# johnmartinsson/differentiable-mel-spectrogram

Hardware: AMD Instinct MI355X
Metric: spectrogram frames/sec (fwd+bwd) (higher is better)
Workload: dtype f32

## Files before the change

differentiable-mel-spectrogram_amd/csrc/dmel_api.cpp:

```cpp
#include "../../include/dmel.h"
#include "dmel_kernels.h"

#include <algorithm>
#include <cmath>
#include <cstdio>
#include <cstdlib>
#include <cstring>
#include <functional>
#include <initializer_list>
#include <map>
#include <mutex>
#include <string>
#include <unordered_set>
#include <vector>

namespace {

thread_local std::string g_err;

dmel_status fail(dmel_status st, const std::string& msg)
{
    g_err = msg;
    return st;
}
// ... 494 lines not shown
                    const bool fin = pc.idx == 0;
                    for (int j = 0; j < 4; ++j) {
                        const int m = 4 * pc.quad + j;
                        lanes[(size_t)ph * 64 + 4 * b + j] = make_int2(8 * k0, (fin && m < M) ? m : -1);
                        merge[(size_t)ph * 64 + 4 * b + j] = (4 * p1 + j) | ((4 * p2 + j) << 8) | (f1 << 16) | (f2 << 17);
                        if (m >= M) continue;
                        for (int st = 0; st < 4 * n4; ++st) {
                            const int f = k0 + st;
                            const float v = (f < tb.F && f >= pc.lo && f < pc.lo + pc.w) ? fb[(size_t)f * M + m] : 0.f;
                            float4& e = b4[base + (size_t)(st / 4) * 64 + 4 * b + j];
                            (st % 4 == 0 ? e.x : st % 4 == 1 ? e.y : st % 4 == 2 ? e.z : e.w) = v;
                        }
                    }
                }
                tb.wl_mg[ph] = mg;
                tb.wl_total4 += n4;
            }
            DMEL_HIP(hipMalloc(&tb.wl_lane, lanes.size() * sizeof(int2)));
            DMEL_HIP(hipMemcpy(tb.wl_lane, lanes.data(), lanes.size() * sizeof(int2), hipMemcpyHostToDevice));
            DMEL_HIP(hipMalloc(&tb.wl_merge, merge.size() * sizeof(int)));
            DMEL_HIP(hipMemcpy(tb.wl_merge, merge.data(), merge.size() * sizeof(int), hipMemcpyHostToDevice));
            DMEL_HIP(hipMalloc(&tb.wl_b4, std::max<size_t>(b4.size(), 64) * sizeof(float4)));
            if (!b4.empty()) DMEL_HIP(hipMemcpy(tb.wl_b4, b4.data(), b4.size() * sizeof(float4), hipMemcpyHostToDevice));
        }
        {
            const int nbpre = dmel::forward_nbpre(N);
            std::vector<float> pre((size_t)waves * 2 * nbpre * 64, 0.f);
            for (int w = 0; w < waves; ++w)
                for (int loc = 0; loc < 2; ++loc) {
                    const int4 tr = ranges[(size_t)w * 2 + loc];
                    const int n = std::min(tr.y, nbpre);
                    tb.pre_groups[w * 2 + loc] = (n + 3) / 4;
                    if (n > 0)
                        std::copy(bfr.begin() + tr.z, bfr.begin() + tr.z + (size_t)n * 64, pre.begin() + ((size_t)(w * 2 + loc) * nbpre) * 64);
                }
            DMEL_HIP(hipMalloc(&tb.ent_pre, pre.size() * sizeof(float)));
            DMEL_HIP(hipMemcpy(tb.ent_pre, pre.data(), pre.size() * sizeof(float), hipMemcpyHostToDevice));
        }
        const size_t nb = std::max<size_t>(bfr.size(), 64);
        DMEL_HIP(hipMalloc(&tb.ent_b, nb * sizeof(float)));
        if (!bfr.empty())
            DMEL_HIP(hipMemcpy(tb.ent_b, bfr.data(), bfr.size() * sizeof(float), hipMemcpyHostToDevice));
        DMEL_HIP(hipMalloc(&tb.tile_ranges, ranges.size() * sizeof(int4)));
        DMEL_HIP(hipMemcpy(tb.tile_ranges, ranges.data(), ranges.size() * sizeof(int4), hipMemcpyHostToDevice));
    }
    auto ins = pl->tables.emplace(N, tb);
    guard.keep = true;
    *out = &ins.first->second;
    return DMEL_OK;
}

constexpr size_t kScratchPartials = 64, kScratchCounter = 64 + 8192, kScratchWin = 8320;
constexpr size_t kScratchPsum = kScratchWin + (size_t)dmel::kMaxNfft * 8;
static_assert(kScratchCounter - kScratchPartials == 1024 * sizeof(double) && dmel::kDotMaxBlocks * sizeof(double) == 4096 &&
              (dmel::kDotMaxBlocks / dmel::kDotGroup) * 64 <= 4096, "scratch layout the ticket tree relies on");

struct Scratch {
    unsigned* handled = nullptr; double* partials = nullptr; unsigned* counter = nullptr; float2* win = nullptr; float* psum = nullptr;
};

size_t scratch_bytes(const dmel_plan* pl, int batch)
{
    const size_t ps = ((size_t)std::max(batch, 1) * pl->nchunks * sizeof(float) + 255) / 256 * 256;
    return kScratchPsum + ps;
}

size_t scratch_bytes_multi(const dmel_plan* pl, int batch, int channels)
{
    return scratch_bytes(pl, batch) + (size_t)(channels - 1) * dmel::kMaxNfft * 8;
}

Scratch carve(void* base, int channels = 1)
{
    unsigned char* b = static_cast<unsigned char*>(base);
    Scratch sc;
    sc.handled = reinterpret_cast<unsigned*>(b);
    sc.partials = reinterpret_cast<double*>(b + kScratchPartials);
    sc.counter = reinterpret_cast<unsigned*>(b + kScratchCounter);
    sc.win = reinterpret_cast<float2*>(b + kScratchWin);
    sc.psum = reinterpret_cast<float*>(b + kScratchPsum + (size_t)(channels - 1) * dmel::kMaxNfft * 8);
    return sc;
}

bool is_capturing(hipStream_t s)
{
    hipStreamCaptureStatus st = hipStreamCaptureStatusNone;
    if (hipStreamIsCapturing(s, &st) != hipSuccess) { (void)hipGetLastError(); return false; }
    return st != hipStreamCaptureStatusNone;
}

dmel_status order_after_last_stream(dmel_plan* pl, hipStream_t s)
{
    if (pl->last_stream_valid && pl->last_stream != s && !is_capturing(s)) {
        if (hipEventRecord(pl->xev, pl->last_stream) == hipSuccess) DMEL_HIP(hipStreamWaitEvent(s, pl->xev, 0));
        else { (void)hipGetLastError(); DMEL_HIP(hipDeviceSynchronize()); }
    }
    pl->last_stream = s;
    pl->last_stream_valid = true;
    return DMEL_OK;
}

dmel_status ensure_own_scratch(dmel_plan* pl, int batch, hipStream_t s, Scratch* sc)
{
    if (!pl->own_scratch || batch > pl->own_scratch_clips) {
        if (is_capturing(s)) return fail(DMEL_ERR_INVALID_ARGUMENT, "plan scratch must grow but the stream is capturing: run one call eagerly first or pass scratch");
        if (pl->own_scratch) { DMEL_HIP(hipDeviceSynchronize()); (void)hipFree(pl->own_scratch); pl->own_scratch = nullptr; pl->own_scratch_clips = 0; }
        const int clips = std::max(batch, pl->cfg.max_batch);
// ... 2018 lines not shown
```

differentiable-mel-spectrogram_amd/csrc/dmel_aux.hip:

```cpp
#include <algorithm>
#include <cstdlib>
#include "dmel_kernels.h"
#include "dmel_ldsfft.h"

namespace dmel {

template <int CTRL> __device__ __forceinline__ double dpp_f64(double v)
{
    const long long b = __builtin_bit_cast(long long, v);
    const int lo = __builtin_amdgcn_mov_dpp((int)b, CTRL, 0xF, 0xF, true);
    const int hi = __builtin_amdgcn_mov_dpp((int)(b >> 32), CTRL, 0xF, 0xF, true);
    return __builtin_bit_cast(double, ((long long)hi << 32) | (unsigned)lo);
}
#ifndef DMEL_DOT_THREADS
#define DMEL_DOT_THREADS 256
#endif
constexpr int kDotThreads = DMEL_DOT_THREADS;
__device__ __forceinline__ double block_sum(double v, double* red4)
{
    v += dpp_f64<0xB1>(v);
    v += dpp_f64<0x4E>(v);
    v += dpp_f64<0x141>(v);
    v += dpp_f64<0x140>(v);
    const int tid = threadIdx.x;
    if ((tid & 15) == 0) red4[tid >> 4] = v;
    __syncthreads();
    double s = 0.0;
    for (int q = 0; q < kDotThreads / 16; ++q) s += red4[q];
    return s;
}

struct AdamConsts { float step, step_size, bc2_sqrt, omb1, omb2, b2, wd, eps; int maximize; };
__device__ __forceinline__ AdamConsts adam_consts(const AdamParams& p, float old_step)
{
    AdamConsts c;
    c.step = old_step + 1.0f;
    const float bc1 = (float)(1.0 - pow(p.beta1, (double)c.step)), bc2 = (float)(1.0 - pow(p.beta2, (double)c.step));
    c.step_size = (float)(p.lr / (double)bc1); c.bc2_sqrt = sqrtf(bc2);
    c.omb1 = (float)(1.0 - p.beta1); c.omb2 = (float)(1.0 - p.beta2); c.b2 = (float)p.beta2; c.wd = (float)p.weight_decay; c.eps = (float)p.eps;
    c.maximize = p.maximize;
    return c;
}
__device__ __forceinline__ void adam_update(const AdamParams& p, const AdamConsts& c, long long i, float g)
{
    const float w = p.param[i];
    if (c.maximize) g = -g;
    if (c.wd != 0.f) g = fmaf(w, c.wd, g);
    float m = p.exp_avg[i], v = p.exp_avg_sq[i];
    m = fmaf(c.omb1, g - m, m);
    v = fmaf(c.b2, v, c.omb2 * g * g);
    const float denom = sqrtf(v) / c.bc2_sqrt + c.eps;
    p.param[i] = w - c.step_size * m / denom;
    p.exp_avg[i] = m; p.exp_avg_sq[i] = v;
}

template <bool GBF16> __device__ __forceinline__ float4 load_g4(const void* g, long long i)
{
    if constexpr (!GBF16) return reinterpret_cast<const float4*>(g)[i];
    else {
        const uint2 v = reinterpret_cast<const uint2*>(g)[i];
        return make_float4(__uint_as_float(v.x << 16), __uint_as_float(v.x & 0xffff0000u),
                           __uint_as_float(v.y << 16), __uint_as_float(v.y & 0xffff0000u));
    }
}
template <bool GBF16> __device__ __forceinline__ float load_g1(const void* g, long long k)
{
    if constexpr (!GBF16) return reinterpret_cast<const float*>(g)[k];
    else return __uint_as_float((unsigned)reinterpret_cast<const unsigned short*>(g)[k] << 16);
}

__device__ __forceinline__ float mailbox_exchange(const MailboxArgs& mb, float local)
{
    const unsigned step = *mb.step + 1u;
    *mb.step = step;
    const unsigned long long mine = ((unsigned long long)step << 32) | __builtin_bit_cast(unsigned, local);
    const int par = (int)(step & 1u) * mb.world;
    for (int r = 0; r < mb.world; ++r)
        __hip_atomic_store(mb.peer_inbox[r] + par + mb.rank, mine, __ATOMIC_RELAXED, __HIP_MEMORY_SCOPE_SYSTEM);
    float sum = 0.f;
    bool ok = true;
    const unsigned long long t_start = __builtin_amdgcn_s_memrealtime();
    for (int r = 0; r < mb.world; ++r) {
        unsigned long long w = 0;
        unsigned spins = 0;
        for (;;) {
            w = __hip_atomic_load(mb.my_inbox + par + r, __ATOMIC_RELAXED, __HIP_MEMORY_SCOPE_SYSTEM);
            if ((unsigned)(w >> 32) == step) break;
            ++spins;
            if (mb.spin_limit && spins >= mb.spin_limit) { ok = false; break; }
            if (mb.timeout_ticks && (spins & 63u) == 0u && __builtin_amdgcn_s_memrealtime() - t_start >= mb.timeout_ticks) { ok = false; break; }
            if (spins < 4096u) __builtin_amdgcn_s_sleep(2); else __builtin_amdgcn_s_sleep(32);
        }
        if (!ok) {
            if (mb.host_error)
                __hip_atomic_store(mb.host_error, ((unsigned long long)step << 32) | (unsigned)r, __ATOMIC_RELAXED, __HIP_MEMORY_SCOPE_SYSTEM);
            return __builtin_nanf("");
        }
        sum += __builtin_bit_cast(float, (unsigned)w);
    }
    return sum;
}

__global__ void __launch_bounds__(64) dmel_mailbox_kernel(float* buf, MailboxArgs mb)
{
    if (threadIdx.x == 0) buf[0] = mailbox_exchange(mb, buf[0]);
}

hipError_t launch_mailbox_allreduce(float* buf, const MailboxArgs& mb, hipStream_t s)
{
    hipLaunchKernelGGL(dmel_mailbox_kernel, dim3(1), dim3(64), 0, s, buf, mb);
    return hipGetLastError();
}

template <bool GBF16, bool MBOX>
__global__ void __launch_bounds__(kDotThreads) dmel_dot_kernel(const void* __restrict__ g, const float* __restrict__ t,
                                                            long long count, double* partials, unsigned* counter,
                                                            int accumulate, float* result, MailboxArgs mb, AdamParams adam)
{
    __shared__ double red4[kDotThreads / 16], red4b[kDotThreads / 16];
    __shared__ int is_last;
    const int tid = threadIdx.x;
    const long long stride = (long long)gridDim.x * kDotThreads;
    double acc = 0.0;
    const uintptr_t galign = GBF16 ? 7 : 15;
    const long long n4 = ((reinterpret_cast<uintptr_t>(g) & galign) | (reinterpret_cast<uintptr_t>(t) & 15)) == 0 ? count / 4 : 0;
    const float4* t4 = reinterpret_cast<const float4*>(t);
    long long i = (long long)blockIdx.x * kDotThreads + tid;
    for (; i + 3 * stride < n4; i += 4 * stride) {
        const float4 a0 = load_g4<GBF16>(g, i), a1 = load_g4<GBF16>(g, i + stride), a2 = load_g4<GBF16>(g, i + 2 * stride), a3 = load_g4<GBF16>(g, i + 3 * stride);
        const float4 b0 = t4[i], b1 = t4[i + stride], b2 = t4[i + 2 * stride], b3 = t4[i + 3 * stride];
        acc += ((double)a0.x * (double)b0.x + (double)a0.y * (double)b0.y) + ((double)a0.z * (double)b0.z + (double)a0.w * (double)b0.w);
        acc += ((double)a1.x * (double)b1.x + (double)a1.y * (double)b1.y) + ((double)a1.z * (double)b1.z + (double)a1.w * (double)b1.w);
        acc += ((double)a2.x * (double)b2.x + (double)a2.y * (double)b2.y) + ((double)a2.z * (double)b2.z + (double)a2.w * (double)b2.w);
        acc += ((double)a3.x * (double)b3.x + (double)a3.y * (double)b3.y) + ((double)a3.z * (double)b3.z + (double)a3.w * (double)b3.w);
    }
    for (; i < n4; i += stride) {
        const float4 a = load_g4<GBF16>(g, i), b = t4[i];
        acc += ((double)a.x * (double)b.x + (double)a.y * (double)b.y) + ((double)a.z * (double)b.z + (double)a.w * (double)b.w);
    }
    for (long long k = n4 * 4 + (long long)blockIdx.x * kDotThreads + tid; k < count; k += stride)
        acc += (double)load_g1<GBF16>(g, k) * (double)t[k];
    const double bsum = block_sum(acc, red4);
    if (tid == 0) {
        __hip_atomic_store(&partials[blockIdx.x], bsum, __ATOMIC_RELAXED, __HIP_MEMORY_SCOPE_AGENT);
        asm volatile("s_waitcnt vmcnt(0)" ::: "memory");
        const unsigned grp = blockIdx.x / kDotGroup, ngroups = (gridDim.x + kDotGroup - 1) / kDotGroup;
        const unsigned gsize = grp + 1 < ngroups ? (unsigned)kDotGroup : gridDim.x - grp * kDotGroup;
        unsigned* gc = dot_group_counters(counter) + 16 * grp;
        bool last = false;
        if (__hip_atomic_fetch_add(gc, 1u, __ATOMIC_RELAXED, __HIP_MEMORY_SCOPE_AGENT) == gsize - 1u) {
            __hip_atomic_store(gc, 0u, __ATOMIC_RELAXED, __HIP_MEMORY_SCOPE_AGENT);
            last = __hip_atomic_fetch_add(counter, 1u, __ATOMIC_RELAXED, __HIP_MEMORY_SCOPE_AGENT) == ngroups - 1u;
        }
        is_last = last;
    }
    __syncthreads();
    if (!is_last) return;
    double sum = 0.0;
    for (int q = tid; q < (int)gridDim.x; q += kDotThreads)
        sum += __hip_atomic_load(&partials[q], __ATOMIC_RELAXED, __HIP_MEMORY_SCOPE_AGENT);
    const double total = block_sum(sum, red4b);
    if (tid == 0) {
        __hip_atomic_store(counter, 0u, __ATOMIC_RELAXED, __HIP_MEMORY_SCOPE_AGENT);
        if constexpr (MBOX) {
            const float all = mailbox_exchange(mb, (float)total);
            result[0] = accumulate ? result[0] + all : all;
        } else {
            result[0] = accumulate ? (float)((double)result[0] + total) : (float)total;
        }
        if (adam.param) {
            const AdamConsts c = adam_consts(adam, *adam.step);
            adam_update(adam, c, 0, result[0]);
            *adam.step = c.step;
        }
    }
}

int dot_blocks_for(long long count, int max_partials)
{
    static const long long per_wg = [] { const char* e = std::getenv("DMEL_DOT_PER_WG"); const long long v = e ? std::atoll(e) : 0; return v >= 1024 ? v : 4096LL; }();
    const long long want = (count + per_wg - 1) / per_wg;
    const long long cap = max_partials < kDotMaxBlocks ? max_partials : kDotMaxBlocks;
    return (int)(want < 1 ? 1 : (want > cap ? cap : want));
}

hipError_t launch_dot(const void* g, int g_bf16, const float* t, long long count, int accumulate, double* partials,
                      unsigned* counter, int max_partials, float* result, hipStream_t s, const MailboxArgs* mb, const AdamParams* fused)
{
    const int blocks = dot_blocks_for(count, max_partials);
    const MailboxArgs none{};
    AdamParams adam{};
    if (fused) adam = *fused;
    const dim3 gr(blocks), bl(kDotThreads);
    if (mb) {
        if (g_bf16) hipLaunchKernelGGL((dmel_dot_kernel<true, true>), gr, bl, 0, s, g, t, count, partials, counter, accumulate, result, *mb, adam);
        else hipLaunchKernelGGL((dmel_dot_kernel<false, true>), gr, bl, 0, s, g, t, count, partials, counter, accumulate, result, *mb, adam);
    } else {
        if (g_bf16) hipLaunchKernelGGL((dmel_dot_kernel<true, false>), gr, bl, 0, s, g, t, count, partials, counter, accumulate, result, none, adam);
        else hipLaunchKernelGGL((dmel_dot_kernel<false, false>), gr, bl, 0, s, g, t, count, partials, counter, accumulate, result, none, adam);
    }
    return hipGetLastError();
}

static_assert(kDotMaxBlocks * sizeof(double) == 4096 && kMaxChannels <= kDotMaxBlocks,
              "the multi dot writes at most kDotMaxBlocks partials: the ticket tree's group counters live in the upper half of the 1024");
template <bool GBF16>
__global__ void __launch_bounds__(kDotThreads) dmel_dot_multi_kernel(const void* __restrict__ g, const float* __restrict__ t, int K,
                                                                  unsigned rows_b, unsigned per_row, int bpc, double* partials,
                                                                  unsigned* counter, int accumulate, float* result)
{
    __shared__ double red4[kDotThreads / 16];
    __shared__ int is_last;
    const int tid = threadIdx.x;
    const int c = blockIdx.x / bpc, j = blockIdx.x - c * bpc;
    const unsigned stride = (unsigned)bpc * kDotThreads;
    double acc = 0.0;
// ... 203 lines not shown
#pragma unroll
            for (int u = 0; u < 4; ++u) {
                const long long i = ((long long)blk * 4 + u) * 256 + tid;
                if (i < n) {
                    p.fb_dense[i] = v[u];
                    if (p.fbT) { const int f = (int)(i / p.M), m = (int)(i % p.M); p.fbT[(size_t)m * p.F + f] = v[u]; }
                }
            }
            return;
        }
        blk -= p.blocks_c;
        const long long f = (long long)blk * 256 + tid;
        if (p.rowpk && f < p.F)
            p.rowpk[f] = make_float4(p.fb[f * p.M], p.M > 1 ? p.fb[f * p.M + 1] : 0.f, __builtin_bit_cast(float, 0), __builtin_bit_cast(float, p.M));
        if (p.ent_h && f < p.M) p.fb_nyq[f] = p.fb[(size_t)(p.F - 1) * p.M + f];
        return;
    }
    const int run = blockIdx.x / kRepackRunSplit, part = blockIdx.x % kRepackRunSplit;
    const int4 tr = p.tile_ranges[run];
    if (tr.y <= 0 || tr.w < 0) return;
    for (int i = part * 256 + tid; i < tr.y * 64; i += 256 * kRepackRunSplit) {
        const int ks = tr.x + i / 64, l = i % 64;
        const int f = 4 * ks + (l >> 4), m = 16 * (tr.w & 0xffff) + (l & 15);
        const float v = (f < p.F && m < p.M) ? p.fb[(size_t)f * p.M + m] : 0.f;
        p.ent_b[tr.z + i] = v;
        if (run < p.runs_group0 && i / 64 < p.nbpre) p.ent_pre[((size_t)run * p.nbpre + i / 64) * 64 + l] = v;
    }
}

hipError_t launch_repack(const RepackParams& p0, hipStream_t s)
{
    RepackParams p = p0;
    const long long n = (long long)p.F * p.M;
    const int NT = (p.M + 15) / 16;
    p.blocks_h = p.ent_h ? (int)(((long long)NT * p.ks32 * 64 + 255) / 256) : 0;
    p.blocks_w = p.wl_b4 ? (int)(((long long)p.wl_total4 * 64 + 255) / 256) : 0;
    p.blocks_c = (int)((n + 1023) / 1024);
    const int blocks_r = (std::max(p.F, p.M) + 255) / 256;
    hipLaunchKernelGGL(dmel_repack_kernel, dim3((unsigned)(p.runs * kRepackRunSplit + p.blocks_h + p.blocks_w + p.blocks_c + blocks_r)), dim3(256), 0, s, p);
    return hipGetLastError();
}

__global__ void __launch_bounds__(128) dmel_naive_kernel(NaiveParams p)
{
    extern __shared__ __attribute__((aligned(16))) unsigned char smem_raw[];
    float* fa = reinterpret_cast<float*>(smem_raw);
    float* fb_ = fa + p.N;
    float* P = fb_ + p.N;
    float* D = P + p.F;
    const int tid = threadIdx.x;
    const int b = blockIdx.x / p.T, t = blockIdx.x % p.T;
    const float* xb = resolve_x(p.x, p.x_ind) + (size_t)b * p.L;
    const bool spec_mode = (p.mode == kSpec || p.mode == kSpecTrain);
    const LamState ls = lam_prologue(p.lam, p.N, blockIdx.x == 0 && tid == 0);
    if (ls.action != kLamRun) {
        if (ls.action == kLamPoison) {
            const int rows = spec_mode ? p.F : p.M;
            for (int rr = tid; rr < rows; rr += blockDim.x) {
                const size_t o = ((size_t)b * rows + rr) * p.T + t;
                if (p.flags & 4u) reinterpret_cast<unsigned short*>(p.out)[o] = 0x7fc0u; else p.out[o] = __builtin_nanf("");
                if (p.tangent) p.tangent[o] = __builtin_nanf("");
            }
        }
        return;
    }
    const float ctan = lam_tangent_scale(ls);
    float mean = 0.f;
    if (p.remove_dc) {
        mean = clip_mean_psum(p.psum, p.nchunks, b, p.L);
    }
    for (int n = tid; n < p.N; n += blockDim.x) {
        const long long i = (long long)t * p.hop - p.N / 2 + n;
        const float v = (i >= 0 && i < p.L) ? (xb[i] - mean) : 0.f;
        const float2 wd = p.win2[n];
        fa[n] = v * wd.x;
        fb_[n] = v * wd.y;
    }
    __syncthreads();
    for (int f = tid; f < p.F; f += blockDim.x) {
        float xr = 0.f, xi = 0.f, yr = 0.f, yi = 0.f;
        for (int n = 0; n < p.N; ++n) {
            const int kn = (int)(((long long)f * n) % p.N);
            float sn, cs;
            sincospif(2.0f * (float)kn / (float)p.N, &sn, &cs);
            xr = fmaf(fa[n], cs, xr); xi = fmaf(-fa[n], sn, xi);
            yr = fmaf(fb_[n], cs, yr); yi = fmaf(-fb_[n], sn, yi);
        }
        P[f] = xr * xr + xi * xi;
        D[f] = 2.f * (xr * yr + xi * yi);
    }
    __syncthreads();
    if (spec_mode) {
        for (int f = tid; f < p.F; f += blockDim.x) {
            const size_t o = ((size_t)b * p.F + f) * p.T + t;
            p.out[o] = P[f];
            if (p.tangent) p.tangent[o] = ctan * D[f];
        }
        return;
    }
    const bool do_log = (p.flags & 1u) != 0;
    for (int m = tid; m < p.M; m += blockDim.x) {
        float mel = 0.f, dmel = 0.f;
        for (int f = 0; f < p.F; ++f) {
            const float c = p.fb[(size_t)f * p.M + m];
            mel = fmaf(c, P[f], mel);
            dmel = fmaf(c, D[f], dmel);
        }
// ... 488 lines not shown
```

differentiable-mel-spectrogram_amd/csrc/dmel_big.hip:

```cpp
#include "dmel_kernels.h"
#include "dmel_ldsfft.h"

namespace dmel {

constexpr int kBigThreads = 1024;

__device__ __forceinline__ float big_wave_sum(float v)
{
    for (int o = 32; o > 0; o >>= 1) v += __shfl_xor(v, o, 64);
    return v;
}

constexpr int kBigBlockLog = 14;
__device__ __forceinline__ int big_block_log(int logM) { return ((logM - kBigBlockLog) & 1) ? kBigBlockLog - 1 : kBigBlockLog; }

template <bool GLOBAL_Z, bool DIT, class TWG, class TWB>
__device__ __forceinline__ void big_fft(float2* Z, int M, int logM, float2* lds_block, int tid, TWG&& twid, TWB&& twid_block)
{
    if constexpr (!GLOBAL_Z) {
        if constexpr (DIT) lds_fft_dit<kBigThreads>(Z, M, logM, tid, twid); else lds_fft_dif<kBigThreads>(Z, M, logM, tid, twid);
    } else {
        const int lgb = big_block_log(logM), ns = logM - lgb, bl = 1 << lgb;
        if constexpr (!DIT) lds_fft_dif_head<kBigThreads>(Z, M, ns, tid, twid, [&](int n) { return Z[n]; }, M);
        for (int blk = 0; blk < (M >> lgb); ++blk) {
// ... 8 lines not shown
    }
}

template <class TWG, class TWB, class LD, class ST>
__device__ __forceinline__ void big_convolve_global(float2* Z, int M, int logM, const float2* __restrict__ hbr, float2* lds_block, int tid,
                                                    TWG&& twid, TWB&& twid_block, LD&& first, ST&& last)
{
    const int lgb = big_block_log(logM), ns = logM - lgb, bl = 1 << lgb;
    lds_fft_dif_head<kBigThreads>(Z, M, ns, tid, twid, first, M);
    for (int blk = 0; blk < (M >> lgb); ++blk) {
        float2* zb = Z + ((size_t)blk << lgb);
        const float2* hb = hbr + ((size_t)blk << lgb);
        for (int i = tid; i < bl; i += kBigThreads) lds_block[i] = zb[i];
        __syncthreads();
        lds_fft_dif<kBigThreads>(lds_block, bl, lgb, tid, twid_block);
        for (int i = tid; i < bl; i += kBigThreads) {
            const float2 v = c_mul(lds_block[i], hb[i]);
            lds_block[i] = make_float2(v.x, -v.y);
        }
        __syncthreads();
        lds_fft_dit<kBigThreads>(lds_block, bl, lgb, tid, twid_block);
        for (int i = tid; i < bl; i += kBigThreads) zb[i] = lds_block[i];
        __syncthreads();
    }
    lds_fft_dit_tail<kBigThreads>(Z, M, ns, tid, twid, last);
}

template <bool GLOBAL_Z>
__global__ void __launch_bounds__(kBigThreads) dmel_big_kernel(BigParams p)
{
    extern __shared__ __attribute__((aligned(16))) unsigned char smem_raw[];
    float2* Z = GLOBAL_Z ? p.zws + (size_t)blockIdx.x * p.Mfft : reinterpret_cast<float2*>(smem_raw);
    const int tid = threadIdx.x, lane = tid & 63, wave = tid >> 6;
    const int N = p.N, M = p.Mfft, F = p.F, sh = 32 - p.logM;
    const int NT = p.split ? N / 2 : N;
    float2* macc = reinterpret_cast<float2*>(smem_raw + (size_t)M * sizeof(float2));
    const int lgb = big_block_log(p.logM), tsh = GLOBAL_Z ? p.logM - lgb : 0, tlen = GLOBAL_Z ? (1 << lgb) : M;
    float2* lds_block = reinterpret_cast<float2*>(smem_raw);
    float2* twa = reinterpret_cast<float2*>(smem_raw + (GLOBAL_Z ? ((size_t)sizeof(float2) << kBigBlockLog) : (size_t)M * sizeof(float2) + (p.split ? (size_t)p.M * sizeof(float2) : 0)));
    float2* twb = twa + 64;
    if (tid < 64) twa[tid] = (128 * tid < (tlen >> 1)) ? p.tw[(128 * tid) << tsh] : make_float2(1.f, 0.f);
    if (tid >= 64 && tid < 192) twb[tid - 64] = (tid - 64 < (tlen >> 1)) ? p.tw[(tid - 64) << tsh] : make_float2(1.f, 0.f);
    auto twid_block = [&](int k) -> float2 { return c_mul(twa[k >> 7], twb[k & 127]); };
    auto twid = [&](int k) -> float2 {
        if (GLOBAL_Z) return p.tw[k];
        return c_mul(twa[k >> 7], twb[k & 127]);
    };
    const bool blue = p.chirp != nullptr;
    const bool pair = (p.mode == kInfer || p.mode == kSpec);
    const bool spec_mode = (p.mode == kSpec || p.mode == kSpecTrain);
    const int tiles = pair ? (p.T + 1) / 2 : p.T;
    const long long units = (long long)p.B * tiles;

    const LamState ls = lam_prologue(p.lam, N, blockIdx.x == 0 && tid == 0);
    if (ls.action != kLamRun) {
        if (ls.action == kLamPoison) {
            const int rows = spec_mode ? F : p.M;
            const long long total = (long long)p.B * rows * p.T;
            for (long long o = (long long)blockIdx.x * kBigThreads + tid; o < total; o += (long long)gridDim.x * kBigThreads) {
                if (p.flags & 4u) reinterpret_cast<unsigned short*>(p.out)[o] = 0x7fc0u; else p.out[o] = __builtin_nanf("");
                if (p.tangent) p.tangent[o] = __builtin_nanf("");
            }
        }
        return;
    }
    const float htan = 0.5f * lam_tangent_scale(ls);
    auto pos = [&](int k) -> unsigned { return blue ? (unsigned)k : (M > 1 ? __brev((unsigned)k) >> sh : 0u); };

    for (long long unit = blockIdx.x; unit < units; unit += gridDim.x) {
        const int b = (int)(unit / tiles), tile = (int)(unit % tiles);
        const int tA = pair ? 2 * tile : tile, tB = tA + 1;
        const float* xb = resolve_x(p.x, p.x_ind) + (size_t)b * p.L;
        float mean = 0.f;
        if (p.remove_dc) {
            mean = clip_mean_psum(p.psum, p.nchunks, b, p.L);
        }
        auto elem = [&](int n) -> float2 {
            const long long ia = (long long)tA * p.hop - N / 2 + n;
            const float va = (ia >= 0 && ia < p.L) ? (xb[ia] - mean) : 0.f;
            const float2 wd = p.win2[n];
            if (pair) {
                const long long ib = ia + p.hop;
                const float vb = (tB < p.T && ib >= 0 && ib < p.L) ? (xb[ib] - mean) : 0.f;
                return make_float2(va * wd.x, vb * wd.x);
            }
            return make_float2(va * wd.x, va * wd.y);
        };
        const int npar = p.split ? 2 : 1;
        for (int par = 0; par < npar; ++par) {
        __syncthreads();
        if (GLOBAL_Z && blue) {
            big_convolve_global(Z, M, p.logM, p.hbr, lds_block, tid, twid, twid_block,
                                [&](int n) -> float2 { return n < N ? c_mul(elem(n), p.chirp[n]) : make_float2(0.f, 0.f); },
                                [&](int k, float2 v) -> float2 { return k < N ? c_mul(make_float2(v.x, -v.y), p.chirp[k]) : v; });
        } else {
        for (int n = tid; n < M; n += kBigThreads) {
            float2 z = make_float2(0.f, 0.f);
            if (n < NT) {
                if (!p.split) z = elem(n);
                else {
                    const float2 za = elem(n), zb = elem(n + NT);
                    z = par == 0 ? make_float2(za.x + zb.x, za.y + zb.y) : c_mul(make_float2(za.x - zb.x, za.y - zb.y), p.wodd[n]);
                }
                if (blue) z = c_mul(z, p.chirp[n]);
            }
            Z[n] = z;
        }
// ... 254 lines not shown
```

differentiable-mel-spectrogram_amd/csrc/dmel_fwd.hip:

```cpp
#include "dmel_kernels.h"
#include "dmel_wavefft.h"


namespace dmel {


#ifndef DMEL_FWD_PART
#define DMEL_FWD_PART 0
#endif
#if DMEL_FWD_PART == 0
__global__ void __launch_bounds__(kThreads) dmel_prep_kernel(PrepParams p)
{
    __shared__ double red[kThreads];
    const int tid = threadIdx.x;
    if (blockIdx.y == (unsigned)p.B) {
        if (blockIdx.x != 0) return;
        const LamState ls = lam_prologue(p.lam, p.N, false);
        if (ls.action != kLamRun) return;
        const float denom = ls.denom;
        const double s2 = (double)ls.s2;
        double s_ww = 0.0, s_wd = 0.0;
        for (int n = tid; n < p.N; n += kThreads) {
            const float d = (float)n - p.center;
            const float t = d / denom;
            float w = expf(-0.5f * (t * t));
            if (p.win_half && (n < p.N / 4 || n >= 3 * p.N / 4)) w = 0.f;
            const double dw = (double)w * (double)d * (double)d * s2;
            p.win2[n] = make_float2(w, (float)dw);
            s_ww += (double)w * (double)w;
            s_wd += (double)w * dw;
        }
        if (!p.normalize) return;
        red[tid] = s_ww; __syncthreads();
        for (int o = kThreads / 2; o > 0; o >>= 1) { if (tid < o) red[tid] += red[tid + o]; __syncthreads(); }
        const double ww = red[0]; __syncthreads();
        red[tid] = s_wd; __syncthreads();
        for (int o = kThreads / 2; o > 0; o >>= 1) { if (tid < o) red[tid] += red[tid + o]; __syncthreads(); }
        const double wd = red[0];
        const double nrm = sqrt(ww);
        for (int n = tid; n < p.N; n += kThreads) {
            const double w = (double)p.win2[n].x;
            const float d = (float)n - p.center;
            const double dwe = w * (double)d * (double)d * s2;
            p.win2[n] = make_float2((float)(w / nrm), (float)(dwe / nrm - w * wd / (nrm * nrm * nrm)));
        }
        return;
    }
    const int b = blockIdx.y, c = blockIdx.x;
    const long long lo = (long long)c * p.chunk;
    long long hi = lo + p.chunk; if (hi > p.L) hi = p.L;
    if (p.lengths) {
        const int lb = p.lengths[b];
        const long long end = (lb >= 1 && lb <= p.L) ? lb : 1;
        if (hi > end) hi = end;
        if (hi < lo) hi = lo;
    }
    const float* xbase = p.x;
    if (p.x_ind) { typedef const float* cfp; xbase = *(const __attribute__((address_space(4))) cfp*)p.x_ind; }
    const float* xb = xbase + (size_t)b * p.L;
    float acc0 = 0.f, acc1 = 0.f, acc2 = 0.f, acc3 = 0.f;
    long long i = lo + tid;
    if (((reinterpret_cast<uintptr_t>(xb + lo)) & 15) == 0) {
        const float4* x4 = reinterpret_cast<const float4*>(xb + lo);
        const long long n4 = (hi - lo) / 4;
        for (long long base = 0; base < n4; base += 4 * kThreads) {
            float4 v[4];
#pragma unroll
            for (int u = 0; u < 4; ++u) { const long long q = base + tid + (long long)u * kThreads; v[u] = x4[q < n4 ? q : n4 - 1]; }
#pragma unroll
            for (int u = 0; u < 4; ++u) {
// ... 353 lines not shown
```

differentiable-mel-spectrogram_amd/csrc/dmel_fwd_body.inc:

```
#if DMEL_FWD_MULTI
#define FWD_BO bo
#define FWD_LAM lam_args
#define FWD_WIN2 win2
#define FWD_LEADER grid_leader
#if DMEL_FWD_BAND
#define FWD_KERNEL dmel_fwd_band_kernel
#else
#define FWD_KERNEL dmel_fwd_multi_kernel
#endif
#else
#define FWD_BO b
#define FWD_LAM p.lam
#define FWD_WIN2 p.win2
#define FWD_LEADER blockIdx.x == 0
#if DMEL_FWD_LEN
#define FWD_KERNEL dmel_fwd_len_kernel
#else
#define FWD_KERNEL dmel_fwd_kernel
#endif
#endif
#if DMEL_FWD_LEN
#define FWD_PARAMS FwdLenParams
#define FWD_LC Lc
#define FWD_INV_L inv_Lc
// ... 227 lines not shown
            bool plain_loads = inside[ti][pass];
#ifdef DMEL_ABLATE
            if (p.flags & 0x4000u) plain_loads = true;
#endif
            if (plain_loads) {
                static_for<0, R>([&](auto aa) {
                    constexpr int a = decltype(aa)::value;
                    xa[ti][pass][a] = buf_f32(rx, (sA + G * a) * 4);
                    if constexpr (PAIR) xb2[ti][pass][a] = buf_f32(rx, (sA + p.hop + G * a) * 4);
                });
            } else {
                static_for<0, R>([&](auto aa) {
                    constexpr int a = decltype(aa)::value;
                    xa[ti][pass][a] = buf_f32(rx, clampi(sA + G * a, FWD_LC - 1) * 4);
                    if constexpr (PAIR) xb2[ti][pass][a] = buf_f32(rx, clampi(sA + p.hop + G * a, FWD_LC - 1) * 4);
                });
            }
        });
    };

#if DMEL_FWD_LEN
    auto fill_rows = [&](int t_first, int t_end, bool pad) {
        const bool do_log = (p.flags & 1u) != 0;
        const bool out_bf16 = (p.flags & 4u) != 0;
        float v = __builtin_nanf(""), tv = v;
        if (pad) {
            const float me = 0.f + p.eps;
            v = do_log ? (WLC ? fast_log(me, p.eps) : logf(me)) : 0.f;
            tv = 0.f;
        }
        if (t_end > p.T) t_end = p.T;
        const int nf = t_end - t_first;
        if (nf <= 0) return;
        for (int idx = tid; idx < p.M * nf; idx += THREADS) {
            const int m = idx / nf, t = t_first + idx % nf;
            const size_t o = ((size_t)b * p.M + m) * p.T + t;
            if (out_bf16) reinterpret_cast<unsigned short*>(p.out)[o] = bf16_bits(v); else p.out[o] = v;
            if (p.tangent) p.tangent[o] = tv;
        }
    };
#endif
    constexpr bool TW1_LDS = g.TW1_OFF != 0;
    constexpr bool TW1_POW = (R >= 16) && !TW1_LDS;
    float mean = 0.f;
    float2 wkeep[WPT];
    float2 wmid = make_float2(1.f, 0.f);
    const float lam_raw = lam_load(FWD_LAM);
    if (!dbg_skip_fft) {
        load_tile(IC<0>{});
        if ((p.flags & kFwdEdgeFirst) && !inside[0][0]) __builtin_amdgcn_s_setprio(2);
        float ps_early = 0.f;
        if (p.remove_dc && p.psum != nullptr) ps_early = (lane < p.nchunks) ? p.psum[(size_t)b * p.nchunks + lane] : 0.f;
        STAMP(1);
        const LamState ls = lam_prologue(FWD_LAM, N, FWD_LEADER && tid == 0, lam_raw);
        if (ls.action != kLamRun) {
            if (ls.action == kLamPoison) {
#if DMEL_FWD_BAND
                const int rows = p.M, nrows = e_hi - e_lo, row0 = e_lo;
#else
                const int rows = IS_SPEC ? F : p.M, nrows = rows;
                constexpr int row0 = 0;
#endif
                const float qn = __builtin_nanf("");
                for (int idx = tid; idx < nrows * FPT * TPW; idx += THREADS) {
                    const int rr = row0 + idx / (FPT * TPW), t = tile0 * FPT + idx % (FPT * TPW);
                    if (t >= p.T) continue;
                    const size_t o = ((size_t)FWD_BO * rows + rr) * p.T + t;
                    if (p.flags & 4u) reinterpret_cast<unsigned short*>(p.out)[o] = 0x7fc0u; else p.out[o] = qn;
                    if (p.tangent) p.tangent[o] = qn;
                }
                if constexpr (TRAINLIKE) {
                    if (p.spec_out) {
                        for (int idx = tid; idx < F * FPT * TPW; idx += THREADS) {
                            const int kk = idx / (FPT * TPW), t = tile0 * FPT + idx % (FPT * TPW);
                            if (t < p.T) p.spec_out[((size_t)b * F + kk) * p.T + t] = qn;
                        }
                    }
                }
            }
            return;
        }
#if DMEL_FWD_LEN
        if (!len_ok || tile0 * FPT >= Tc) {
            fill_rows(tile0 * FPT, (tile0 + TPW) * FPT, len_ok);
            return;
        }
#endif
        if constexpr (WPF > 1) {
            if (tid < 4) fctr[tid] = 0u;
            __syncthreads();
        }
        if constexpr (TRAINLIKE || MODE == kSpecTrain) {
            if (wave == 0) { const float h = 0.5f * lam_tangent_scale(ls); if (lane == 0) red[kRedTan] = h; }
        }
        if constexpr (TW2_LDS) { if (tid < R * C) tw2l[tid] = p.tw2[tid]; }
        if constexpr (TW1_LDS) {
            constexpr int n16 = (R - 1) * G / 2;
            for (int i = tid; i < n16; i += THREADS)
                reinterpret_cast<float4*>(smem_raw + g.TW1_OFF)[i] = reinterpret_cast<const float4*>(p.tw1 + G)[i];
        }
        if constexpr (SPLIT && !IS_SPEC) {
            constexpr int first = 2 * F, count = SS * 2 - first;
            static_assert(count >= 0, "slot stride covers PD[0 .. N/2]");
            if constexpr (count > 0) {
                constexpr int CP = 1 << (ilog2(count - 1 > 0 ? count - 1 : 1) + 1);
                static_assert(count <= CP, "slot padding fits the zeroing loop");
#ifdef DMEL_ABLATE
// ... 1010 lines not shown
```

differentiable-mel-spectrogram_amd/csrc/dmel_kernels.h:

```cpp
#pragma once
#include <hip/hip_runtime.h>
#include <stdint.h>

namespace dmel {

constexpr int kWave = 64;
constexpr int kThreads = 256;
constexpr int kMaxChunks = 64;
constexpr int kMaxFastNfft = 16384;
constexpr int kMaxNfft = 16384;
constexpr int kMinFastNfft = 32;

__device__ __forceinline__ unsigned short bf16_bits(float v) { return __builtin_bit_cast(unsigned short, (__bf16)v); }

enum Mode : int { kTrain = 0, kInfer = 1, kSpec = 2, kSpecTrain = 3,
                  kTrainH = 4,
                  kTrainW = 5,
                  kTrainWW = 6 };
constexpr bool mode_wlc(int mode) { return mode == kTrainW || mode == kTrainWW; }
#ifndef DMEL_WLC_4096
#define DMEL_WLC_4096 0
#endif
#ifndef DMEL_WLC_512
#define DMEL_WLC_512 0
#endif
constexpr bool wlc_size(int n_fft) { return (DMEL_WLC_512 && n_fft == 512) || n_fft == 1024 || n_fft == 2048 || (DMEL_WLC_4096 && n_fft == 4096); }
constexpr int kWlMaxPhases = 8;
constexpr int kHsplitMinNfft = 64, kHsplitMaxNfft = 4096;
constexpr int hsplit_plane_stride(int n_fft) { return n_fft / 2 + 8; }

constexpr unsigned kLamFirst = 1u, kLamLast = 2u, kLamQuiet = 4u;
constexpr unsigned kLamRing = 256;
struct LamArgs {
    const float* dev;
    float val;
    int n_expected;
    unsigned role;
    unsigned* exec_counter;
    unsigned* handled;
    unsigned long long* host_seen;
    unsigned long long* host_error;
    unsigned* dot_counter;
};

constexpr int kDotGroup = 16, kDotMaxBlocks = 512;
__host__ __device__ inline unsigned* dot_group_counters(unsigned* ticket_word)
{
    return reinterpret_cast<unsigned*>(reinterpret_cast<unsigned char*>(ticket_word) - 4096);
}

constexpr int kMaxChannels = 8;
constexpr unsigned kLamMultiStride = kLamRing + 1;
__host__ __device__ inline LamArgs lam_for_channel(const LamArgs& base, int c, int slot, unsigned roles, const float* vals)
{
    LamArgs la = base;
    if (la.dev) la.dev += c;
    la.val = vals[c];
    la.role = (roles >> (4 * slot)) & 15u;
    if (la.handled) la.handled += 2 * c;
    if (la.exec_counter) la.exec_counter += c;
    if (la.host_seen) la.host_seen += (size_t)c * kLamMultiStride;
    if (la.host_error) la.host_error += (size_t)c * kLamMultiStride;
    if (slot != 0) la.dot_counter = nullptr;
    return la;
}

enum LamAction : int { kLamRun = 0, kLamSkip = 1, kLamPoison = 2 };
struct LamState {
    float lam, a, denom;
    float s2;
    int e2;
    int action;
};

#if defined(__HIPCC__)
__device__ __forceinline__ float mean_quotient(float sum, int L, float inv)
{
    const float fl = (float)L;
    const float q = sum * inv;
    return fmaf(fmaf(-q, fl, sum), inv, q);
}
__device__ __forceinline__ float clip_mean_psum(const float* psum, int nchunks, int b, int L)
{
    double s = 0.0;
    for (int c = 0; c < nchunks; ++c) s += (double)psum[(size_t)b * nchunks + c];
    return (float)(s / (double)L);
}

__device__ __forceinline__ int lam_n_fft(float a)
{
    const float prod = a * 6.0f;
    const int x = __builtin_amdgcn_readfirstlane((int)prod);
    const int v = x - 1;
    const int bits = v < 0 ? 1 : (v == 0 ? 0 : 32 - __builtin_clz((unsigned)v));
    return bits > 30 ? 0x40000000 : (1 << bits);
}

__device__ __forceinline__ float lam_load(const LamArgs& la)
{
    typedef const __attribute__((address_space(4))) float cfloat;
    float v = la.val;
    if (la.dev) v = *(cfloat*)la.dev;
    return v;
}

__device__ __forceinline__ LamState lam_prologue(const LamArgs& la, int n_launch, bool leader, float lam_value)
{
    LamState st;
    st.lam = lam_value;
    st.a = __builtin_fabsf(st.lam);
    st.denom = st.a + 1e-15f;
    int e = __builtin_amdgcn_readfirstlane(st.a > 1e-30f ? __builtin_amdgcn_frexp_expf(st.a) : 1);
    e = e < -30 ? -30 : (e > 30 ? 30 : e);
    st.e2 = 2 * e;
    st.s2 = __builtin_bit_cast(float, (127 - 2 * e) << 23);
    const bool match = la.n_expected == 0 || lam_n_fft(st.a) == n_launch;
    st.action = match ? kLamRun : kLamSkip;
    if (la.role & kLamQuiet) return st;
    if (la.role & kLamFirst) {
        if (leader) {
            if (la.exec_counter && la.host_seen) {
                const unsigned num = __hip_atomic_fetch_add(la.exec_counter, 1u, __ATOMIC_RELAXED, __HIP_MEMORY_SCOPE_AGENT) + 1u;
                __hip_atomic_store(la.host_seen + (num % kLamRing), ((unsigned long long)num << 32) | __builtin_bit_cast(unsigned, st.lam),
                                   __ATOMIC_RELAXED, __HIP_MEMORY_SCOPE_SYSTEM);
                if (la.handled) la.handled[1] = num;
            }
            if (la.dot_counter) {
                *la.dot_counter = 0u;
                unsigned* gc = dot_group_counters(la.dot_counter);
                for (int g2 = 0; g2 < kDotMaxBlocks / kDotGroup; ++g2) gc[16 * g2] = 0u;
            }
            if (la.handled) la.handled[0] = match ? 1u : 0u;
        }
    } else if (match && leader && la.handled) {
        la.handled[0] = 1u;
    }
    if (!match && (la.role & kLamLast)) {
        const unsigned prior = ((la.role & kLamFirst) || !la.handled) ? 0u : la.handled[0];
        if (!prior) {
            st.action = kLamPoison;
            if (leader && la.host_error) {
                const unsigned num = la.handled ? la.handled[1] : 0u;
                __hip_atomic_store(la.host_error, ((unsigned long long)num << 32) | __builtin_bit_cast(unsigned, st.lam),
                                   __ATOMIC_RELAXED, __HIP_MEMORY_SCOPE_SYSTEM);
            }
        }
    }
    return st;
}

__device__ __forceinline__ LamState lam_prologue(const LamArgs& la, int n_launch, bool leader)
{
    return lam_prologue(la, n_launch, leader, lam_load(la));
}

__device__ __forceinline__ float lam_tangent_scale(const LamState& st)
{
    const double den = (double)st.denom;
    const double sg = st.lam > 0.f ? 1.0 : (st.lam < 0.f ? -1.0 : 0.0);
    const float c = (float)(sg * __builtin_ldexp(1.0, st.e2) / (den * den * den));
    return (c == c && __builtin_fabsf(c) < 3.0e38f) ? c : 0.f;
}
#endif

template <int N> struct FftPlan;
constexpr int kPairLds = 0, kPairBperm = 1, kPairPlane = 2;
template <> struct FftPlan<32>   { static constexpr int R = 4,  C = 2, PASSES = 1, WAVES = 4, NBPRE = 4, MINW = 4, PAIRING = 0, SPLIT = 0; };
template <> struct FftPlan<64>   { static constexpr int R = 8,  C = 1, PASSES = 1, WAVES = 4, NBPRE = 4, MINW = 4, PAIRING = 0, SPLIT = 0; };
template <> struct FftPlan<128>  { static constexpr int R = 8,  C = 2, PASSES = 1, WAVES = 4, NBPRE = 8, MINW = 4, PAIRING = 0, SPLIT = 0; };
template <> struct FftPlan<256>  { static constexpr int R = 16, C = 1, PASSES = 1, WAVES = 4, NBPRE = 12, MINW = 4, PAIRING = 0, SPLIT = 0; };
template <> struct FftPlan<512>  { static constexpr int R = 16, C = 2, PASSES = 1, WAVES = 4, NBPRE = 20, MINW = 4, PAIRING = 0, SPLIT = 0; };
template <> struct FftPlan<1024> { static constexpr int R = 32, C = 1, PASSES = 1, WAVES = 8, NBPRE = 20, MINW = 4, PAIRING = 1, SPLIT = 1; };
template <> struct FftPlan<2048> { static constexpr int R = 32, C = 2, PASSES = 1, WAVES = 8, NBPRE = 40, MINW = 4, PAIRING = 1, SPLIT = 1; };
template <> struct FftPlan<4096> { static constexpr int R = 64, C = 1, PASSES = 1, WAVES = 8, NBPRE = 40, MINW = 2, PAIRING = 1, SPLIT = 1; };
template <> struct FftPlan<8192> { static constexpr int R = 64, C = 2, PASSES = 1, WAVES = 8, NBPRE = 40, MINW = 2, PAIRING = 2, SPLIT = 1; };
template <> struct FftPlan<16384> { static constexpr int R = 64, C = 4, PASSES = 1, WAVES = 8, NBPRE = 40, MINW = 2, PAIRING = 2, SPLIT = 1; };

template <int N, bool PAIR> struct FftPlanSel : FftPlan<N> {};
template <> struct FftPlanSel<1024, true> { static constexpr int R = 16, C = 4, PASSES = 1, WAVES = 8, NBPRE = 20, MINW = 4, PAIRING = 0, SPLIT = 0; };
constexpr bool mode_pairs(int mode) { return mode == kInfer || mode == kSpec; }
template <int N, bool PAIR, bool WL> struct FftPlanSel3 : FftPlanSel<N, PAIR> {};
#ifndef DMEL_WL512_WAVES
#define DMEL_WL512_WAVES 8
#endif
template <> struct FftPlanSel3<512, false, true> { static constexpr int R = 16, C = 2, PASSES = 1, WAVES = DMEL_WL512_WAVES, NBPRE = 20, MINW = 4, PAIRING = 1, SPLIT = 1; };

constexpr unsigned kFwdEdgeFirst = 0x40u;
int forward_resident_workgroups(int n_fft, int mode);
constexpr int kWinLdsMaxNfft = 4096;
constexpr int kRedBytes = 160;
constexpr int kRedTan = 32;
struct FftGeom {
    int N, R, C, G, FPW, PASSES, WAVES, NLOC, THREADS, SLOTS, MT, EX_STRIDE, SLOT_STRIDE_F2, NBPRE, MINW, LDS_BYTES, AUX_OFF, RED_OFF, WIN_LDS;
    int PAIRING, SPLIT, WIN_SYM, WPF, PLANE_PAD;
    int TW1_OFF;
};

constexpr int ex_stride(int G, int C) { return G + (G >= 32 ? C : 1); }
constexpr int z_index_host(int k, int R, int C) { return C == 1 ? k : k + (k / (R * R)) * 4; }
constexpr int slot_stride_f2(int N, int R, int C, int pairing = 0, int split = 0, bool wl = false)
{
    const int G = N / R;
    const int a = R * ex_stride(G, C) * (split ? 4 : 8);
    const int b = (z_index_host(pairing ? N / 2 : N - 1, R, C) + 1) * 8;
    const int need = a > b ? a : b;
    if (wl) return ((need + 127) / 128 * 128 + 64) / 8;
// ... 282 lines not shown
```

Baseline: 215.3 million.

## Replace dot-kernel ticket-tree completion with tagged-slot spin wait in last block

```diff
diff --git a/differentiable-mel-spectrogram_amd/csrc/dmel_api.cpp b/differentiable-mel-spectrogram_amd/csrc/dmel_api.cpp
--- a/differentiable-mel-spectrogram_amd/csrc/dmel_api.cpp
+++ b/differentiable-mel-spectrogram_amd/csrc/dmel_api.cpp
@@ -570,7 +570,7 @@
 
 constexpr size_t kScratchPartials = 64, kScratchCounter = 64 + 8192, kScratchWin = 8320;
 constexpr size_t kScratchPsum = kScratchWin + (size_t)dmel::kMaxNfft * 8;
-static_assert(kScratchCounter - kScratchPartials == 1024 * sizeof(double) && dmel::kDotMaxBlocks * sizeof(double) == 4096 &&
+static_assert(kScratchCounter - kScratchPartials == (size_t)dmel::kDotAreaBytes && kScratchWin - kScratchCounter >= 8 && dmel::kDotMaxBlocks * sizeof(double) == 4096 &&
               (dmel::kDotMaxBlocks / dmel::kDotGroup) * 64 <= 4096, "scratch layout the ticket tree relies on");
 
 struct Scratch {
diff --git a/differentiable-mel-spectrogram_amd/csrc/dmel_aux.hip b/differentiable-mel-spectrogram_amd/csrc/dmel_aux.hip
--- a/differentiable-mel-spectrogram_amd/csrc/dmel_aux.hip
+++ b/differentiable-mel-spectrogram_amd/csrc/dmel_aux.hip
@@ -16,6 +16,7 @@
 #define DMEL_DOT_THREADS 256
 #endif
 constexpr int kDotThreads = DMEL_DOT_THREADS;
+constexpr unsigned long long kDotWaitTicks = 200000000ull;
 __device__ __forceinline__ double block_sum(double v, double* red4)
 {
     v += dpp_f64<0xB1>(v);
@@ -118,8 +119,9 @@
                                                             int accumulate, float* result, MailboxArgs mb, AdamParams adam)
 {
     __shared__ double red4[kDotThreads / 16], red4b[kDotThreads / 16];
-    __shared__ int is_last;
+    __shared__ int timed_out;
     const int tid = threadIdx.x;
+    const unsigned seq = *(const __attribute__((address_space(4))) unsigned*)(counter + 1);
     const long long stride = (long long)gridDim.x * kDotThreads;
     double acc = 0.0;
     const uintptr_t galign = GBF16 ? 7 : 15;
@@ -140,28 +142,38 @@
     }
     for (long long k = n4 * 4 + (long long)blockIdx.x * kDotThreads + tid; k < count; k += stride)
         acc += (double)load_g1<GBF16>(g, k) * (double)t[k];
+    if (tid == 0) timed_out = 0;
     const double bsum = block_sum(acc, red4);
+    typedef __attribute__((address_space(1))) unsigned long long gu64;
+    gu64* slots = (gu64*)partials;
+    const unsigned long long tag = (unsigned long long)dot_tag(seq) << 32;
     if (tid == 0) {
-        __hip_atomic_store(&partials[blockIdx.x], bsum, __ATOMIC_RELAXED, __HIP_MEMORY_SCOPE_AGENT);
-        asm volatile("s_waitcnt vmcnt(0)" ::: "memory");
-        const unsigned grp = blockIdx.x / kDotGroup, ngroups = (gridDim.x + kDotGroup - 1) / kDotGroup;
-        const unsigned gsize = grp + 1 < ngroups ? (unsigned)kDotGroup : gridDim.x - grp * kDotGroup;
-        unsigned* gc = dot_group_counters(counter) + 16 * grp;
-        bool last = false;
-        if (__hip_atomic_fetch_add(gc, 1u, __ATOMIC_RELAXED, __HIP_MEMORY_SCOPE_AGENT) == gsize - 1u) {
-            __hip_atomic_store(gc, 0u, __ATOMIC_RELAXED, __HIP_MEMORY_SCOPE_AGENT);
-            last = __hip_atomic_fetch_add(counter, 1u, __ATOMIC_RELAXED, __HIP_MEMORY_SCOPE_AGENT) == ngroups - 1u;
-        }
-        is_last = last;
-    }
-    __syncthreads();
-    if (!is_last) return;
+        const unsigned long long bits = __builtin_bit_cast(unsigned long long, bsum);
+        __hip_atomic_store(slots + 2 * blockIdx.x, tag | (bits & 0xffffffffull), __ATOMIC_RELAXED, __HIP_MEMORY_SCOPE_AGENT);
+        __hip_atomic_store(slots + 2 * blockIdx.x + 1, tag | (bits >> 32), __ATOMIC_RELAXED, __HIP_MEMORY_SCOPE_AGENT);
+    }
+    if (blockIdx.x != gridDim.x - 1) return;
     double sum = 0.0;
-    for (int q = tid; q < (int)gridDim.x; q += kDotThreads)
-        sum += __hip_atomic_load(&partials[q], __ATOMIC_RELAXED, __HIP_MEMORY_SCOPE_AGENT);
-    const double total = block_sum(sum, red4b);
+    const unsigned long long t_start = __builtin_amdgcn_s_memrealtime();
+    for (int q = tid; q < (int)gridDim.x; q += kDotThreads) {
+        unsigned long long lo, hi;
+        bool ok = true;
+        for (unsigned spins = 1;; ++spins) {
+            lo = __hip_atomic_load(slots + 2 * q, __ATOMIC_RELAXED, __HIP_MEMORY_SCOPE_AGENT);
+            hi = __hip_atomic_load(slots + 2 * q + 1, __ATOMIC_RELAXED, __HIP_MEMORY_SCOPE_AGENT);
+            if (((lo ^ tag) >> 32) == 0 && ((hi ^ tag) >> 32) == 0) break;
+            if ((spins & 15u) == 0u && __builtin_amdgcn_s_memrealtime() - t_start >= kDotWaitTicks) { ok = false; break; }
+            __builtin_amdgcn_s_sleep(1);
+        }
+        __hip_atomic_store(slots + 2 * q, 0ull, __ATOMIC_RELAXED, __HIP_MEMORY_SCOPE_AGENT);
+        __hip_atomic_store(slots + 2 * q + 1, 0ull, __ATOMIC_RELAXED, __HIP_MEMORY_SCOPE_AGENT);
+        if (!ok) timed_out = 1;
+        sum += __builtin_bit_cast(double, (hi << 32) | (lo & 0xffffffffull));
+    }
+    double total = block_sum(sum, red4b);
     if (tid == 0) {
-        __hip_atomic_store(counter, 0u, __ATOMIC_RELAXED, __HIP_MEMORY_SCOPE_AGENT);
+        if (timed_out) total = __builtin_nan("");
+        counter[1] = seq + 1u;
         if constexpr (MBOX) {
             const float all = mailbox_exchange(mb, (float)total);
             result[0] = accumulate ? result[0] + all : all;
@@ -471,7 +483,7 @@
     const int b = blockIdx.x / p.T, t = blockIdx.x % p.T;
     const float* xb = resolve_x(p.x, p.x_ind) + (size_t)b * p.L;
     const bool spec_mode = (p.mode == kSpec || p.mode == kSpecTrain);
-    const LamState ls = lam_prologue(p.lam, p.N, blockIdx.x == 0 && tid == 0);
+    const LamState ls = lam_prologue(p.lam, p.N, blockIdx.x == 0, tid, (int)blockDim.x);
     if (ls.action != kLamRun) {
         if (ls.action == kLamPoison) {
             const int rows = spec_mode ? p.F : p.M;
diff --git a/differentiable-mel-spectrogram_amd/csrc/dmel_big.hip b/differentiable-mel-spectrogram_amd/csrc/dmel_big.hip
--- a/differentiable-mel-spectrogram_amd/csrc/dmel_big.hip
+++ b/differentiable-mel-spectrogram_amd/csrc/dmel_big.hip
@@ -84,7 +84,7 @@
     const int tiles = pair ? (p.T + 1) / 2 : p.T;
     const long long units = (long long)p.B * tiles;
 
-    const LamState ls = lam_prologue(p.lam, N, blockIdx.x == 0 && tid == 0);
+    const LamState ls = lam_prologue(p.lam, N, blockIdx.x == 0, tid, (int)blockDim.x);
     if (ls.action != kLamRun) {
         if (ls.action == kLamPoison) {
             const int rows = spec_mode ? F : p.M;
diff --git a/differentiable-mel-spectrogram_amd/csrc/dmel_fwd.hip b/differentiable-mel-spectrogram_amd/csrc/dmel_fwd.hip
--- a/differentiable-mel-spectrogram_amd/csrc/dmel_fwd.hip
+++ b/differentiable-mel-spectrogram_amd/csrc/dmel_fwd.hip
@@ -15,7 +15,7 @@
     const int tid = threadIdx.x;
     if (blockIdx.y == (unsigned)p.B) {
         if (blockIdx.x != 0) return;
-        const LamState ls = lam_prologue(p.lam, p.N, false);
+        const LamState ls = lam_prologue(p.lam, p.N, false, 0, 1);
         if (ls.action != kLamRun) return;
         const float denom = ls.denom;
         const double s2 = (double)ls.s2;
diff --git a/differentiable-mel-spectrogram_amd/csrc/dmel_fwd_body.inc b/differentiable-mel-spectrogram_amd/csrc/dmel_fwd_body.inc
--- a/differentiable-mel-spectrogram_amd/csrc/dmel_fwd_body.inc
+++ b/differentiable-mel-spectrogram_amd/csrc/dmel_fwd_body.inc
@@ -303,7 +303,7 @@
         float ps_early = 0.f;
         if (p.remove_dc && p.psum != nullptr) ps_early = (lane < p.nchunks) ? p.psum[(size_t)b * p.nchunks + lane] : 0.f;
         STAMP(1);
-        const LamState ls = lam_prologue(FWD_LAM, N, FWD_LEADER && tid == 0, lam_raw);
+        const LamState ls = lam_prologue(FWD_LAM, N, (FWD_LEADER), tid, THREADS, lam_raw);
         if (ls.action != kLamRun) {
             if (ls.action == kLamPoison) {
 #if DMEL_FWD_BAND
diff --git a/differentiable-mel-spectrogram_amd/csrc/dmel_kernels.h b/differentiable-mel-spectrogram_amd/csrc/dmel_kernels.h
--- a/differentiable-mel-spectrogram_amd/csrc/dmel_kernels.h
+++ b/differentiable-mel-spectrogram_amd/csrc/dmel_kernels.h
@@ -44,10 +44,13 @@
 };
 
 constexpr int kDotGroup = 16, kDotMaxBlocks = 512;
+constexpr int kDotAreaBytes = 8192;
+static_assert(kDotMaxBlocks * 16 == kDotAreaBytes, "one 16-byte slot per workgroup of dmel_dot_kernel");
 __host__ __device__ inline unsigned* dot_group_counters(unsigned* ticket_word)
 {
     return reinterpret_cast<unsigned*>(reinterpret_cast<unsigned char*>(ticket_word) - 4096);
 }
+__host__ __device__ inline unsigned dot_tag(unsigned seq) { return 0xFFF40000u | (seq & 0x3FFFFu); }
 
 constexpr int kMaxChannels = 8;
 constexpr unsigned kLamMultiStride = kLamRing + 1;
@@ -104,8 +107,9 @@
     return v;
 }
 
-__device__ __forceinline__ LamState lam_prologue(const LamArgs& la, int n_launch, bool leader, float lam_value)
-{
+__device__ __forceinline__ LamState lam_prologue(const LamArgs& la, int n_launch, bool leader_wg, int tid, int nthreads, float lam_value)
+{
+    const bool leader = leader_wg && tid == 0;
     LamState st;
     st.lam = lam_value;
     st.a = __builtin_fabsf(st.lam);
@@ -125,12 +129,12 @@
                                    __ATOMIC_RELAXED, __HIP_MEMORY_SCOPE_SYSTEM);
                 if (la.handled) la.handled[1] = num;
             }
-            if (la.dot_counter) {
-                *la.dot_counter = 0u;
-                unsigned* gc = dot_group_counters(la.dot_counter);
-                for (int g2 = 0; g2 < kDotMaxBlocks / kDotGroup; ++g2) gc[16 * g2] = 0u;
-            }
             if (la.handled) la.handled[0] = match ? 1u : 0u;
+        }
+        if (leader_wg && la.dot_counter) {
+            uint4* area = reinterpret_cast<uint4*>(reinterpret_cast<unsigned char*>(la.dot_counter) - kDotAreaBytes);
+            for (int q = tid; q < kDotAreaBytes / 16; q += nthreads) area[q] = make_uint4(0u, 0u, 0u, 0u);
+            if (tid == 0) *la.dot_counter = 0u;
         }
     } else if (match && leader && la.handled) {
         la.handled[0] = 1u;
@@ -149,9 +153,9 @@
     return st;
 }
 
-__device__ __forceinline__ LamState lam_prologue(const LamArgs& la, int n_launch, bool leader)
-{
-    return lam_prologue(la, n_launch, leader, lam_load(la));
+__device__ __forceinline__ LamState lam_prologue(const LamArgs& la, int n_launch, bool leader_wg, int tid, int nthreads)
+{
+    return lam_prologue(la, n_launch, leader_wg, tid, nthreads, lam_load(la));
 }
 
 __device__ __forceinline__ float lam_tangent_scale(const LamState& st)
```

New measurement: 218.8 million (median of 6 runs). No clear change (+1.6%).
